# Fan-Luo/Legal-RAG

Hardware: AMD Instinct MI355X
Metric: queries/sec + Recall@10 (hybrid top-10) on UCC-en (higher is better)
Workload: dtype f32 dense (long batches: fp16 first pass, candidates re-scored in f32) / f64 bm25+fusion; 1 GPU; UCC-en 591 chunks, dense(768-d FlatIP)+BM25 hybrid fusion top-10 (BASELINE configs[1]); unique_queries=1168, top_k=10, fusion=rrf_norm_blend w=0.6/0.4 alpha=0.5 rrf_k=60 min_final=0.2

## Files before the change

legal-rag_amd/csrc/dense_tail.hip:

```cpp
#include "bm25_core.hpp"
#include "dense_dot.hpp"
#include "fuse_core.hpp"

#include <cfloat>
#include <cstdlib>

namespace amdr {

__global__ __launch_bounds__(64) void dense_select_fuse_kernel(amdr_fuse_params_t P, const float* __restrict__ S,
                                                               long ldS, long n, int nq, int kd, int cap,
                                                               float* __restrict__ fin_scores,
                                                               long long* __restrict__ fin_ids, ChanIn c0, ChanIn c1,
                                                               int max_out, long long* __restrict__ out_ids,
                                                               double* __restrict__ out_vals, int* __restrict__ out_mask,
                                                               int* __restrict__ out_count) {
  extern __shared__ __attribute__((aligned(16))) unsigned char smem[];
  C32* buf = reinterpret_cast<C32*>(smem);
  const int lane = threadIdx.x, sl = lane & 31;
  const int q = 2 * blockIdx.x + (lane >> 5);
  const bool has_q = q < nq;
  FusePre pre;
  pre.dense_bm25(c1, q, sl, has_q);
  C32 out = C32::pad();
  int got = select_row_pair_any(S, ldS, n, q, has_q, kd, lane, buf, out);
  if (got < 0) pair_rows_staged(S, ldS, n, 2 * blockIdx.x, nq, kd, cap, buf, lane, true, out, got);
  const bool v = sl < got;
  if (has_q && sl < kd) topk_store(out, v, sl, fin_scores + (size_t)q * kd, fin_ids + (size_t)q * kd);
  pre.dense(out, v);
  fuse_packed_body<32, true>(P, c0, c1, ChanIn::none(), nq, max_out, out_ids, out_vals, out_mask, out_count, pre, blockIdx.x * 2);
}

template <int V>
__device__ __forceinline__ int select_row_pair_margin(const float* __restrict__ S, long ldS, long n, int q, bool has_q, int k,
                                                      float margin, int lane, C32* scratch, C32& out, int& need) {
  const float* row = S + (size_t)q * ldS;
  const int j = lane & 31;
  f32x4 blk[V / 4];
#pragma unroll
  for (int u = 0; u < V / 4; ++u) {
    const long c0 = 128L * u + 4 * j;
    const f32x4 z = {0.f, 0.f, 0.f, 0.f};
    blk[u] = (has_q && c0 < ldS) ? __builtin_nontemporal_load(reinterpret_cast<const f32x4*>(row + c0)) : z;
  }
  u32 sk[V];
#pragma unroll
  for (int u = 0; u < V / 4; ++u)
#pragma unroll
    for (int e = 0; e < 4; ++e) {
      const long r = 128L * u + 4 * j + e;
      sk[4 * u + e] = (has_q && r < n) ? ord32(blk[u][e]) : 0u;
    }
  K32 lb;
  lb.c = 0u;
#pragma unroll
  for (int v = 0; v < V; ++v) lb.c = sk[v] > lb.c ? sk[v] : lb.c;
  const K32 sorted_best = wave_sortN_desc<K32, 32>(lb, lane);
  const int kk = (k - 1 < 31 ? k - 1 : 31);
  auto half_lane = [&](int x, int pos) -> int {
    const int a = __builtin_amdgcn_readlane(x, pos), b = __builtin_amdgcn_readlane(x, 32 + pos);
    return (lane & 32) ? b : a;
  };
  const u32 T = (u32)half_lane((int)sorted_best.c, kk);
  auto gather = [&](u32 Te, C32& c) -> int {
    int mine = 0;
#pragma unroll
    for (int v = 0; v < V; ++v) mine += (sk[v] >= Te) ? 1 : 0;
    int incl = mine;
    incl += __builtin_amdgcn_update_dpp(0, incl, 0x111, 0xf, 0xf, false);
    incl += __builtin_amdgcn_update_dpp(0, incl, 0x112, 0xf, 0xf, false);
    incl += __builtin_amdgcn_update_dpp(0, incl, 0x114, 0xf, 0xf, false);
    incl += __builtin_amdgcn_update_dpp(0, incl, 0x118, 0xf, 0xf, false);
    incl += __builtin_amdgcn_update_dpp(0, incl, 0x142, 0xa, 0xf, false);
    const int cnt = half_lane(incl, 31);
    if (cnt > 32) return -1;
    int at = (lane & 32) + incl - mine;
#pragma unroll
    for (int v = 0; v < V; ++v) {
      if (sk[v] >= Te) {
        C32 e;
        e.c = ((u64)sk[v] << 32) | (u64)(0xffffffffu - (u32)(128 * (v >> 2) + 4 * j + (v & 3)));
        scratch[at++] = e;
      }
    }
    wave_lds_fence();
    c = (j < cnt) ? scratch[lane] : C32::pad();
    c = wave_sortN_desc<C32, 32>(c, lane);
    wave_lds_fence();
    return cnt;
  };
  const u32 Te1 = T > 1u ? T : 1u;
  C32 c;
  int cnt = gather(Te1, c);
  if (cnt < 0) return -1;
  u32 cut = 1u;
  if (cnt > kk) {
    const float tk_f = __int_as_float(half_lane(__float_as_int(c.score()), kk));
    cut = ord32(tk_f - margin);
    cut = cut > 1u ? cut : 1u;
  }
  if (cut < Te1) {
    cnt = gather(cut, c);
    if (cnt < 0) return -1;
    need = cnt;
  } else {
    const unsigned long long m = __ballot(j < cnt && (u32)(c.c >> 32) >= cut);
    need = __popcll((lane & 32) ? (m >> 32) : (m & 0xffffffffull));
  }
  out = c;
  return cnt;
}

template <bool FUSE, int D128>
__global__ __launch_bounds__(64) void dense_hi_select_fuse_kernel(amdr_fuse_params_t P, const float* __restrict__ S, long ldS, long n,
                                                                  int nq, int kd, const float* __restrict__ X,
                                                                  const float* __restrict__ Q, int d,
                                                                  const float* __restrict__ eps, float margin_scale,
                                                                  float* __restrict__ fin_scores, long long* __restrict__ fin_ids,
                                                                  ChanIn c0, ChanIn c1, int max_out,
                                                                  long long* __restrict__ out_ids, double* __restrict__ out_vals,
                                                                  int* __restrict__ out_mask, int* __restrict__ out_count,
                                                                  unsigned int* __restrict__ fallbacks) {
  extern __shared__ __attribute__((aligned(16))) unsigned char smem[];
  C32* buf = reinterpret_cast<C32*>(smem);
  const int lane = threadIdx.x, sl = lane & 31, half = lane >> 5;
  const int q = 2 * blockIdx.x + half;
  const bool has_q = q < nq;
  FusePre pre;
  pre.have[0] = pre.have[1] = true;
  pre.have[2] = false;
  pre.id[1] = -1;
  pre.s[1] = 0.0;
  if (FUSE && has_q && sl < c1.k) {
    pre.id[1] = c1.ids[(size_t)q * c1.k + sl];
    pre.s[1] = chan_score(c1, q, sl);
  }
  const float e_q = has_q ? eps[q] : 0.f;
  const float margin = 2.f * e_q * margin_scale;
  bool exact_all = has_q && !(margin == margin && margin <= FLT_MAX);
  f32x4 qv[D128];
#pragma unroll
  for (int u = 0; u < D128; ++u) {
    const f32x4 z = {0.f, 0.f, 0.f, 0.f};
    qv[u] = has_q ? __builtin_nontemporal_load(reinterpret_cast<const f32x4*>(Q + (size_t)q * d + 128 * u + 4 * sl)) : z;
  }
  auto half_sum = [&](float v) -> float {
    v = dpp_add<0x111, 0xf>(v);
    v = dpp_add<0x112, 0xf>(v);
    v = dpp_add<0x114, 0xf>(v);
    v = dpp_add<0x118, 0xf>(v);
    v = dpp_add<0x142, 0xa>(v);
    const float s0 = __int_as_float(__builtin_amdgcn_readlane(__float_as_int(v), 31));
    const float s1 = __int_as_float(__builtin_amdgcn_readlane(__float_as_int(v), 63));
    return half ? s1 : s0;
  };
  auto row_load = [&](long r, f32x4 (&xv)[D128]) {
    const float* xr = X + (size_t)r * d + 4 * sl;
#pragma unroll
    for (int u = 0; u < D128; ++u) xv[u] = *reinterpret_cast<const f32x4*>(xr + 128 * u);
  };
  auto row_fma = [&](const f32x4 (&xv)[D128]) -> float {
    float acc = 0.f;
#pragma unroll
    for (int u = 0; u < D128; ++u)
#pragma unroll
      for (int e = 0; e < 4; ++e) acc = fmaf(xv[u][e], qv[u][e], acc);
    return half_sum(acc);
  };
  auto row_dot = [&](long r) -> float {
    f32x4 xv[D128];
    row_load(r, xv);
    return row_fma(xv);
  };
  C32 out = C32::pad();
  int need = 0, got = 0;
  {
    const float mg = (has_q && !exact_all) ? margin : 0.f;
    if (n <= 256)
      got = select_row_pair_margin<8>(S, ldS, n, q, has_q, kd, mg, lane, buf, out, need);
    else if (n <= 512)
      got = select_row_pair_margin<16>(S, ldS, n, q, has_q, kd, mg, lane, buf, out, need);
    else if (n <= 640)
      got = select_row_pair_margin<20>(S, ldS, n, q, has_q, kd, mg, lane, buf, out, need);
    else
      got = select_row_pair_margin<32>(S, ldS, n, q, has_q, kd, mg, lane, buf, out, need);
    exact_all = exact_all || (has_q && got < 0);
    if (exact_all) need = 0;
  }
  if (__any(exact_all)) {
    const unsigned long long fbm = __ballot(exact_all && sl == 0);
    if (lane == 0 && fallbacks) atomicAdd(fallbacks, (unsigned int)__popcll(fbm));
    const C32 keep = out;
    const int keep_need = need, keep_got = got;
    float* xs = const_cast<float*>(S);
    for (long r = 0; r < n; ++r) {
      const float v = row_dot(r);
      if (exact_all && sl == 0) xs[(size_t)q * ldS + r] = v;
    }
    __threadfence_block();
    C32 o2 = C32::pad();
    int g2 = select_row_pair_any(xs, ldS, n, q, has_q && exact_all, kd, lane, buf, o2);
    if (g2 < 0) pair_rows_staged(xs, ldS, n, 2 * blockIdx.x, nq, kd, 128, buf, lane, exact_all, o2, g2);
    if (exact_all) {
      out = o2;
      got = g2 < kd ? g2 : kd;
      need = 0;
    } else {
      out = keep;
      got = keep_got;
      need = keep_need;
    }
  }
  const int steps = __builtin_amdgcn_readfirstlane(max(__shfl(need, 0), __shfl(need, 32)));
  float mine_exact = 0.f;
  const int my_id = (int)out.id();
  for (int c = 0; c < steps; c += 2) {
    const int c1 = c + 1 < 32 ? c + 1 : 31;
    const int ra0 = __builtin_amdgcn_readlane(my_id, c), ra1 = __builtin_amdgcn_readlane(my_id, 32 + c);
    const int rb0 = __builtin_amdgcn_readlane(my_id, c1), rb1 = __builtin_amdgcn_readlane(my_id, 32 + c1);
    const bool la = c < need, lb = c + 1 < need;
    f32x4 xa[D128], xb[D128];
    row_load(la ? (long)(half ? ra1 : ra0) : 0, xa);
    row_load(lb ? (long)(half ? rb1 : rb0) : 0, xb);
    const float va = row_fma(xa), vb = row_fma(xb);
    if (la && sl == c) mine_exact = va;
    if (lb && sl == c + 1) mine_exact = vb;
  }
  if (need > 0) {
    C32 c = (sl < need) ? C32::make(mine_exact, (u32)out.id()) : C32::pad();
    c = wave_sortN_desc<C32, 32>(c, lane);
    out = c;
    got = need < kd ? need : kd;
  }
  const bool v = sl < got && sl < kd;
  if (has_q && sl < kd) topk_store(out, v, sl, fin_scores + (size_t)q * kd, fin_ids + (size_t)q * kd);
  if (FUSE) {
    pre.dense(out, v);
    fuse_packed_body<32, true>(P, c0, c1, ChanIn::none(), nq, max_out, out_ids, out_vals, out_mask, out_count, pre, blockIdx.x * 2);
  }
}

struct SmallArgs {
  const long long* term_ptr;
  const int* post_doc;
  const double* post_w;
  const double* idf;
  long n_terms, n_docs;
  const int* q_terms;
  const long long* q_ptr;
  int kb, cap, slab, use_select;
  double* bm_scores;
  long long* bm_ids;
  const float* X;
  const float* Q;
  long n_rows;
  int d, rows_per_block, blocks_per_query;
  float* S;
  long ldS;
  int kd, cap_sel;
  float* d_scores;
  long long* d_ids;
  int* ticket;
};

__device__ __forceinline__ int small_arrive(int* counter, int lane) {
  asm volatile("s_waitcnt vmcnt(0)" ::: "memory");
  int t = 0;
  if (lane == 0) {
    __builtin_amdgcn_fence(__ATOMIC_RELEASE, "agent");
    asm volatile("s_waitcnt vmcnt(0)" ::: "memory");
    t = __hip_atomic_fetch_add(counter, 1, __ATOMIC_RELAXED, __HIP_MEMORY_SCOPE_AGENT);
  }
  return __builtin_amdgcn_readfirstlane(t);
}
__device__ __forceinline__ void small_acquire(int* counter, int lane) {
  if (lane == 0) __hip_atomic_store(counter, 0, __ATOMIC_RELAXED, __HIP_MEMORY_SCOPE_AGENT);
  __builtin_amdgcn_fence(__ATOMIC_ACQUIRE, "agent");
  asm volatile("s_waitcnt vmcnt(0)" ::: "memory");
}

template <int NVT>
__global__ __launch_bounds__(256) void hybrid_small_kernel(SmallArgs A, amdr_fuse_params_t P, ChanIn c0, ChanIn c1, int nq,
                                                           int max_out, long long* __restrict__ out_ids,
                                                           double* __restrict__ out_vals, int* __restrict__ out_mask,
                                                           int* __restrict__ out_count) {
  extern __shared__ __attribute__((aligned(16))) unsigned char smem[];
  const int q = blockIdx.y, role = blockIdx.x;
  const int lane = threadIdx.x & 63, wave = threadIdx.x >> 6;
  int* rows_done = A.ticket + q;
  int* lists_done = A.ticket + 32 + q;
  const int sl = lane & 31;
  C32 dense_mine = C32::pad();
  bool have_dense = false, dense_valid = false;
  if (role == 0) {
    if (wave != 0) return;
    bm25_block_query<1, NVT>(A.term_ptr, A.post_doc, A.post_w, A.idf, A.n_terms, A.n_docs, A.q_terms, A.q_ptr, nq, A.kb,
                             A.cap, A.slab, A.use_select, nullptr, nullptr, A.bm_scores, A.bm_ids, q, 0, smem);
  } else {
    const long r0 = (long)(role - 1) * A.rows_per_block;
    long r1 = r0 + A.rows_per_block;
    if (r1 > A.n_rows) r1 = A.n_rows;
    for (long r = r0 + wave; r < r1; r += 4) {
      const float acc = dense_row_dot(A.X + (size_t)r * A.d, A.Q + (size_t)q * A.d, A.d, lane);
      if (lane == 63) A.S[(size_t)q * A.ldS + r] = acc;
    }
    asm volatile("s_waitcnt vmcnt(0)" ::: "memory");
    __syncthreads();
    if (wave != 0) return;
    if (small_arrive(rows_done, lane) != A.blocks_per_query - 2) return;
    small_acquire(rows_done, lane);
    C32* buf = reinterpret_cast<C32*>(smem);
    const float* row = A.S + (size_t)q * A.ldS;
    const long n = A.n_rows;
    WaveTopK<C32> tk;
    tk.init(buf, A.cap_sel, A.kd);
    const int got = select_row_any(row, 0, n, A.kd, lane, tk.buf);
    if (got >= 0)
      tk.cnt = got;
    else
      wave_topk_sweep(tk, row, 0, n, lane);
    wave_lds_fence();
    const bool v = lane < 32 && sl < tk.cnt;
    const C32 mine = v ? tk.buf[sl] : C32::pad();
    if (lane < A.kd) topk_store(mine, v, lane, A.d_scores + (size_t)q * A.kd, A.d_ids + (size_t)q * A.kd);
    dense_mine = mine;
    dense_valid = v;
    have_dense = true;
    wave_lds_fence();
  }
  if (small_arrive(lists_done, lane) != 1) return;
  small_acquire(lists_done, lane);
  long long dense_id = -1;
  double dense_s = 0.0;
  if (!have_dense && lane < 32 && sl < A.kd) {
    dense_id = A.d_ids[(size_t)q * A.kd + sl];
    dense_s = dense_id >= 0 ? (double)A.d_scores[(size_t)q * A.kd + sl] : 0.0;
  }
  FusePre pre;
  pre.dense_bm25(c1, q, sl, lane < 32);
  if (have_dense) {
    pre.dense(dense_mine, dense_valid);
  } else {
    pre.id[0] = dense_id;
    pre.s[0] = dense_s;
  }
  fuse_packed_body<32, true>(P, c0, c1, ChanIn::none(), q + 1, max_out, out_ids, out_vals, out_mask, out_count, pre, q);
}

bool dense_select_fuse_applies(long n, int slabs, int m, int kd, int kb) {
  const char* e = getenv("AMDR_DENSE_FUSE");
  if (e && e[0] == '0') return false;
  return slabs == 1 && n >= 1 && n <= 1024 && kd >= 1 && kd <= 32 && kb >= 0 && kd + kb <= 32 && m >= 1;
}

int dense_select_fuse_launch(const FuseTail& t, int q0, const float* S, long ldS, long n, int m, int kd, int cap,
                             float* fin_scores, int64_t* fin_ids, hipStream_t st) {
  const FuseTailArgs a = fuse_tail_args(t, q0, kd, nullptr, nullptr);
  hipLaunchKernelGGL(dense_select_fuse_kernel, dim3((m + 1) / 2), dim3(64), (size_t)cap * sizeof(C32), st, *t.p, S, ldS, n,
                     m, kd, cap, fin_scores, (long long*)fin_ids, a.c0, a.c1, a.mo, a.ids, a.vals, a.mask, a.count);
  AMDR_HIP(hipGetLastError());
  return AMDR_OK;
}

template <bool FUSE, class... Args>
static void hi_select_dispatch(int d, int m, size_t lds, hipStream_t st, Args... args) {
#define AMDR_HSF(D) \
  hipLaunchKernelGGL((dense_hi_select_fuse_kernel<FUSE, D>), dim3((m + 1) / 2), dim3(64), lds, st, args...)
  switch (d >> 7) {
    case 1: AMDR_HSF(1); break;
    case 2: AMDR_HSF(2); break;
    case 3: AMDR_HSF(3); break;
    case 4: AMDR_HSF(4); break;
    case 5: AMDR_HSF(5); break;
    case 6: AMDR_HSF(6); break;
    case 7: AMDR_HSF(7); break;
    default: AMDR_HSF(8); break;
  }
#undef AMDR_HSF
}

int dense_hi_select_launch(const FuseTail* t, int q0, const float* S, long ldS, long n, int m, int kd, const float* X,
                           const float* Q, int d, const float* eps, float* fin_scores, int64_t* fin_ids,
                           unsigned int* fallbacks, hipStream_t st) {
  const char* ms = getenv("AMDR_DENSE_SMALL_HI_MARGIN");
  const float margin_scale = ms ? (float)atof(ms) : 1.f;
  const size_t lds = 128 * sizeof(C32);
  const amdr_fuse_params_t P0{};
  const FuseTailArgs a = t ? fuse_tail_args(*t, q0, kd, nullptr, nullptr)
                           : FuseTailArgs{ChanIn::none(), ChanIn::none(), 0, nullptr, nullptr, nullptr, nullptr};
  if (t)
    hi_select_dispatch<true>(d, m, lds, st, *t->p, S, ldS, n, m, kd, X, Q, d, eps, margin_scale, fin_scores,
                             (long long*)fin_ids, a.c0, a.c1, a.mo, a.ids, a.vals, a.mask, a.count, fallbacks);
  else
    hi_select_dispatch<false>(d, m, lds, st, P0, S, ldS, n, m, kd, X, Q, d, eps, margin_scale, fin_scores,
                              (long long*)fin_ids, a.c0, a.c1, a.mo, a.ids, a.vals, a.mask, a.count, fallbacks);
  AMDR_HIP(hipGetLastError());
  return AMDR_OK;
}

bool hybrid_small_applies(long n_dense, long n_bm25, int nslabs, int nq, int kd, int kb) {
  const char* e = getenv("AMDR_HYBRID_SMALL");
  if (e && e[0] == '0') return false;
  return nq >= 1 && nq <= 4 && n_dense >= 1 && n_dense <= kSelectRowsMax && n_bm25 >= 1 && nslabs == 1 && kd >= 1 && kb >= 1 &&
         kd + kb <= 32;
}

static int hybrid_small_rows(long n, int nq) {
  static const int pinned = [] {
    const char* e = getenv("AMDR_HYBRID_SMALL_ROWS");
    int r = e ? atoi(e) : 0;
    if (r <= 0) return 0;
    if (r < 4) r = 4;
    if (r > 64) r = 64;
    return (r + 3) / 4 * 4;
  }();
  if (pinned) return pinned;
  return n * nq <= 2560 ? 16 : 32;
}

int hybrid_small_launch(const DenseRaw& dr, const Bm25Raw& br, const float* Q, const int* q_terms, const long long* q_ptr,
                        int nq, int kd, int kb, const amdr_fuse_params_t& P, const int64_t* dense_row2uid,
                        const int64_t* bm25_row2uid, float* dense_scores, int64_t* dense_ids, double* bm25_scores,
                        int64_t* bm25_ids, int64_t* out_ids, double* out_vals, int32_t* out_mask, int32_t* out_count,
                        hipStream_t st) {
  SmallArgs A;
  A.term_ptr = br.term_ptr;
  A.post_doc = br.post_doc;
  A.post_w = br.post_w;
  A.idf = br.idf;
  A.n_terms = br.n_terms;
  A.n_docs = br.n_docs;
  A.q_terms = q_terms;
  A.q_ptr = q_ptr;
  A.kb = kb;
  A.cap = br.cap;
  A.slab = br.slab;
  A.use_select = br.select_on ? 1 : 0;
  A.bm_scores = bm25_scores;
  A.bm_ids = (long long*)bm25_ids;
  A.X = dr.X;
  A.Q = Q;
  A.d = dr.d;
  A.n_rows = dr.n;
  A.rows_per_block = hybrid_small_rows(dr.n, nq);
  const int dense_blocks = (int)((dr.n + A.rows_per_block - 1) / A.rows_per_block);
  A.blocks_per_query = 1 + dense_blocks;
  A.S = dr.S;
  A.ldS = dr.ld;
  A.kd = kd;
  int cap_sel = topk_cap(kd);
  if (cap_sel < 128) cap_sel = 128;
  A.cap_sel = cap_sel;
  A.d_scores = dense_scores;
  A.d_ids = (long long*)dense_ids;
  A.ticket = br.ticket;
  size_t lds = br.lds;
  if (lds < (size_t)cap_sel * sizeof(C32)) lds = (size_t)cap_sel * sizeof(C32);
  const int mo = kd + kb;
  ChanIn c0{nullptr, nullptr, (const long long*)dense_row2uid, kd, 0};
  ChanIn c1{(const long long*)bm25_ids, (const void*)bm25_scores, (const long long*)bm25_row2uid, kb, 1};
#define AMDR_HS_LAUNCH(NVT)                                                                                        \
  hipLaunchKernelGGL((hybrid_small_kernel<NVT>), dim3(A.blocks_per_query, nq), dim3(256), lds, st, A, P, c0, c1, nq, mo, \
                     (long long*)out_ids, out_vals, out_mask, out_count)
  const int nv = br.nvt;
  if (nv <= 4) AMDR_HS_LAUNCH(4);
  else if (nv <= 8) AMDR_HS_LAUNCH(8);
  else if (nv <= 10) AMDR_HS_LAUNCH(10);
  else if (nv <= 16) AMDR_HS_LAUNCH(16);
  else if (nv <= 20) AMDR_HS_LAUNCH(20);
  else AMDR_HS_LAUNCH(32);
#undef AMDR_HS_LAUNCH
  AMDR_HIP(hipGetLastError());
  return AMDR_OK;
}

}

using namespace amdr;

extern "C" {

int amdr_hybrid_small_device(amdr_dense_t* dense, amdr_bm25_t* bm25, const float* Q_dev, const int32_t* q_terms_dev,
                             const int64_t* q_ptr_dev, int32_t nq, int32_t kd, int32_t kb, const amdr_fuse_params_t* p,
                             const int64_t* dense_row2uid, const int64_t* bm25_row2uid, float* dense_scores_dev,
                             int64_t* dense_ids_dev, double* bm25_scores_dev, int64_t* bm25_ids_dev, int64_t* out_ids,
                             double* out_vals, int32_t* out_mask, int32_t* out_count, void* stream) {
  AMDR_REQUIRE(dense && bm25, "hybrid_small: null index handle");
  AMDR_REQUIRE(p != nullptr, "hybrid_small: null params");
  AMDR_REQUIRE(p->method >= 0 && p->method <= AMDR_FUSE_WEIGHTED_SUM, "hybrid_small: method=%d", p->method);
  AMDR_REQUIRE(nq >= 0 && kd >= 1 && kd <= AMDR_MAX_K && kb >= 1 && kb <= AMDR_MAX_K, "hybrid_small: bad sizes");
  if (nq == 0) return AMDR_OK;
  AMDR_REQUIRE(Q_dev && q_terms_dev && q_ptr_dev, "hybrid_small: null query buffers");
  AMDR_REQUIRE(dense_scores_dev && dense_ids_dev && bm25_scores_dev && bm25_ids_dev, "hybrid_small: null channel lists");
  AMDR_REQUIRE(out_ids && out_vals && out_mask && out_count, "hybrid_small: null output");
  int64_t nd = 0, nb = 0;
  int rc;
  if ((rc = amdr_dense_ntotal(dense, &nd))) return rc;
  if ((rc = amdr_bm25_ndocs(bm25, &nb))) return rc;
  AMDR_REQUIRE(kd <= nd || nd == 0, "hybrid_small: kd=%d > %lld rows", kd, (long long)nd);
  bool one = false;
  if (nd >= 1 && nb >= 1 && nq <= 4 && dense_device_of(dense) >= 0) {
    std::lock_guard<std::mutex> gd(dense_mutex(dense));
    std::lock_guard<std::mutex> gb(bm25_mutex(bm25));
    AMDR_HIP(hipSetDevice(dense_device_of(dense)));
    Bm25Raw br;
    if ((rc = bm25_small_raw(bm25, nq, kb, &br))) return rc;
    if (hybrid_small_applies((long)nd, (long)nb, br.nslabs, nq, kd, kb)) {
      DenseRaw dr;
      if ((rc = dense_small_raw(dense, nq, &dr))) return rc;
      one = true;
      rc = hybrid_small_launch(dr, br, Q_dev, q_terms_dev, (const long long*)q_ptr_dev, nq, kd, kb, *p, dense_row2uid,
                               bm25_row2uid, dense_scores_dev, dense_ids_dev, bm25_scores_dev, bm25_ids_dev, out_ids,
                               out_vals, out_mask, out_count, (hipStream_t)stream);
    }
  }
  if (one) return rc;
  if ((rc = amdr_bm25_search_device(bm25, q_terms_dev, q_ptr_dev, nq, kb, bm25_scores_dev, bm25_ids_dev, stream))) return rc;
  return amdr_dense_search_fuse_device(dense, Q_dev, nq, kd, p, dense_row2uid, bm25_ids_dev, bm25_scores_dev, kb,
                                       bm25_row2uid, dense_scores_dev, dense_ids_dev, out_ids, out_vals, out_mask,
                                       out_count, stream);
}

}
```

legal-rag_amd/csrc/fuse_core.hpp:

```cpp
#pragma once
#include "common.hpp"
#include "topk.hpp"

#include <cmath>

namespace amdr {

__device__ __forceinline__ double wave_min(double v) { return wave_allmin_f64(v); }
__device__ __forceinline__ double wave_max(double v) { return wave_allmax_f64(v); }
__device__ __forceinline__ void lds_sync() {
  __builtin_amdgcn_fence(__ATOMIC_ACQ_REL, "wavefront");
  __builtin_amdgcn_wave_barrier();
}

struct ChanIn {
  const long long* ids;
  const void* scores;
  const long long* row2uid;
  int k;
  int is_f64;
  __host__ __device__ static ChanIn none() { return ChanIn{nullptr, nullptr, nullptr, 0, 0}; }
};

__device__ __forceinline__ double chan_score(const ChanIn& c, int qi, int j) {
  size_t off = (size_t)qi * c.k + j;
  return c.is_f64 ? ((const double*)c.scores)[off] : (double)((const float*)c.scores)[off];
}
__device__ __forceinline__ long long chan_uid(const ChanIn& c, int qi, int j) {
  long long id = c.ids[(size_t)qi * c.k + j];
  if (id >= 0 && c.row2uid) id = c.row2uid[id];
  return id;
}

struct FuseCtx {
  double rmn, rmx;
  bool rdeg, wrrf;
  double w[3], lo[3], hi[3];
};
template <class ScoreAt>
__device__ __forceinline__ void fuse_eval(const amdr_fuse_params_t& P, const FuseCtx& X, double t, const int (&pos)[3],
                                          ScoreAt&& score_at, double (&val)[AMDR_FUSE_NVALS], int& mk) {
  const double rrf_norm = X.rdeg ? 0.0 : (t - X.rmn) / (X.rmx - X.rmn);
  double nrm[3], raw[3], wt[3];
  mk = 0;
#pragma unroll
  for (int c = 0; c < 3; ++c) {
    const int p = pos[c];
    nrm[c] = 0.0;
    raw[c] = 0.0;
    if (p >= 0) {
      mk |= (1 << c);
      const double s = score_at(c, p);
      nrm[c] = (X.hi[c] - X.lo[c] < 1e-12) ? 0.0 : (s - X.lo[c]) / (X.hi[c] - X.lo[c]);
      const double wc = X.wrrf ? X.w[c] : 1.0;
      raw[c] = wc * (1.0 / (double)(P.rrf_k + p + 1));
    }
    wt[c] = X.w[c] * nrm[c];
  }
  const double wsum = (wt[0] + wt[1]) + wt[2];
  double score, con[3] = {0.0, 0.0, 0.0};
  if (P.method == AMDR_FUSE_WEIGHTED_SUM) {
    score = wsum;
#pragma unroll
    for (int c = 0; c < 3; ++c) con[c] = wt[c];
  } else if (P.method == AMDR_FUSE_RRF || P.method == AMDR_FUSE_WRRF) {
    score = rrf_norm;
    const double mass = score;
    if (!(mass <= 0.0 || t <= 1e-18)) {
#pragma unroll
      for (int c = 0; c < 3; ++c)
        if (pos[c] >= 0) con[c] = mass * raw[c] / t;
    }
  } else {
    score = P.alpha * rrf_norm + (1.0 - P.alpha) * wsum;
#pragma unroll
    for (int c = 0; c < 3; ++c) con[c] = 0.0 + (1.0 - P.alpha) * wt[c];
    const double mass = P.alpha * rrf_norm;
    if (!(mass <= 0.0 || t <= 1e-18)) {
#pragma unroll
      for (int c = 0; c < 3; ++c)
        if (pos[c] >= 0) con[c] = con[c] + mass * raw[c] / t;
    }
  }
  val[AMDR_FV_SCORE] = score;
  val[AMDR_FV_RRF_NORM] = rrf_norm;
  val[AMDR_FV_WSUM] = wsum;
  val[AMDR_FV_NORM_DENSE] = nrm[0];
  val[AMDR_FV_NORM_BM25] = nrm[1];
  val[AMDR_FV_NORM_COLBERT] = nrm[2];
  val[AMDR_FV_CONTRIB_DENSE] = con[0];
  val[AMDR_FV_CONTRIB_BM25] = con[1];
  val[AMDR_FV_CONTRIB_COLBERT] = con[2];
}

struct FusePre {
  bool have[3];
  long long id[3];
  double s[3];
  __device__ __forceinline__ void dense_bm25(const ChanIn& c1, int q, int sl, bool live) {
    have[0] = have[1] = true;
    have[2] = false;
    id[1] = -1;
    s[1] = 0.0;
    if (live && sl < c1.k) {
      id[1] = c1.ids[(size_t)q * c1.k + sl];
      s[1] = chan_score(c1, q, sl);
    }
  }
  __device__ __forceinline__ void dense(const C32& c, bool valid) {
    id[0] = valid ? c.id() : -1ll;
    s[0] = valid ? (double)c.score() : 0.0;
  }
  __device__ __forceinline__ void bm25(const C64& c, bool valid) {
    id[1] = valid ? c.idv : -1ll;
    s[1] = valid ? unord64(c.key) : 0.0;
  }
};
template <int W, bool PRE>
__device__ __forceinline__ void fuse_packed_body(const amdr_fuse_params_t& P, const ChanIn& c0, const ChanIn& c1,
                                                 const ChanIn& c2, int nq, int max_out, long long* __restrict__ out_ids,
                                                 double* __restrict__ out_vals, int* __restrict__ out_mask,
                                                 int* __restrict__ out_count, const FusePre& pre, int qbase) {
  constexpr int G = 64 / W;
  __shared__ long long s_uid[G][W];
  __shared__ double s_sc[G][W];
  __shared__ double s_chs[G][3][W];
  __shared__ int s_pos[G][3][W];
  const int lane = threadIdx.x, seg = lane / W, sl = lane % W;
  const int qi = qbase + seg;
  const bool live = qi < nq;
  const ChanIn ch[3] = {c0, c1, c2};
  const double w[3] = {P.w_dense, P.w_bm25, P.w_colbert};
  const unsigned long long seg_bits = (W == 64) ? ~0ull : (((1ull << (W & 63)) - 1ull) << (seg * W));
  long long* uid = s_uid[seg];
  double* sc = s_sc[seg];

  int n[3] = {0, 0, 0};
  double lo[3] = {INFINITY, INFINITY, INFINITY}, hi[3] = {-INFINITY, -INFINITY, -INFINITY};
  long long my_uid[3] = {-1, -1, -1};
#pragma unroll
  for (int c = 0; c < 3; ++c) {
    if (ch[c].k == 0) continue;
    const int j = sl;
    const bool inr = live && j < ch[c].k;
    long long id = -1;
    double s = 0.0;
    if (PRE && pre.have[c]) {
      if (inr) {
        id = pre.id[c];
        s = pre.s[c];
      }
    } else if (inr) {
      id = ch[c].ids[(size_t)qi * ch[c].k + j];
      s = chan_score(ch[c], qi, j);
    }
    const bool has = inr && id >= 0;
    if (!has) s = 0.0;
    if (has && ch[c].row2uid) id = ch[c].row2uid[id];
    my_uid[c] = has ? id : -1;
    s_chs[seg][c][sl] = s;
    const unsigned long long hm = __ballot(has) & seg_bits;
    n[c] = __popcll(hm);
    const double nxt = __shfl_down(s, 1);
    const bool in_order = !(has && sl + 1 < n[c]) || s >= nxt;
    const bool prefix = hm == (seg_bits & ((n[c] >= 64 ? ~0ull : ((1ull << n[c]) - 1ull)) << (seg * W)));
    if (__ballot(!in_order || !prefix) == 0ull) {
      const int first = seg * W, last = seg * W + (n[c] > 0 ? n[c] - 1 : 0);
      const double top = __shfl(s, first), bot = __shfl(s, last);
      hi[c] = n[c] > 0 ? top : -(double)INFINITY;
      lo[c] = n[c] > 0 ? bot : (double)INFINITY;
    } else {
      lo[c] = seg_allmin_f64<W>(has ? s : (double)INFINITY);
      hi[c] = seg_allmax_f64<W>(has ? s : -(double)INFINITY);
    }
  }

  int U = 0;
#pragma unroll
  for (int c = 0; c < 3; ++c) {
    if (ch[c].k == 0) continue;
    const int U0 = U;
    const bool v = sl < n[c];
    const long long my = my_uid[c];
    int f = -1;
    int u_end = 0;
#pragma unroll
    for (int g = 0; g < G; ++g) {
      const int ug = __builtin_amdgcn_readlane(U0, g * W);
      u_end = ug > u_end ? ug : u_end;
    }
    for (int u0 = 0; u0 < u_end; u0 += 4) {
      long long e[4];
#pragma unroll
      for (int i = 0; i < 4; ++i) e[i] = uid[(u0 + i) & (W - 1)];
#pragma unroll
      for (int i = 0; i < 4; ++i) f = (u0 + i < U0 && e[i] == my) ? u0 + i : f;
    }
    f = v ? f : -1;
    const bool isnew = v && f < 0;
    const unsigned long long m = __ballot(isnew) & seg_bits;
    const unsigned long long lt = m & ((1ull << lane) - 1ull);
    const int idx = isnew ? U + __popcll(lt) : f;
    if (isnew) {
      uid[idx] = my;
      s_pos[seg][0][idx] = -1;
      s_pos[seg][1][idx] = -1;
      s_pos[seg][2][idx] = -1;
    }
    lds_sync();
    if (v) s_pos[seg][c][idx] = sl;
    U += __popcll(m);
    lds_sync();
  }

  const bool wrrf = (P.method == AMDR_FUSE_WRRF);
  const int u = sl;
  const bool act = u < U;
  int pp[3] = {-1, -1, -1};
  double t = 0.0;
  if (act) {
#pragma unroll
    for (int c = 0; c < 3; ++c) {
      pp[c] = s_pos[seg][c][u];
      if (pp[c] >= 0) {
        const double wc = wrrf ? w[c] : 1.0;
        const double v = wc * (1.0 / (double)(P.rrf_k + pp[c] + 1));
        t = t + v;
      }
    }
  }
  FuseCtx X;
  X.rmn = seg_allmin_f64<W>(act ? t : (double)INFINITY);
  X.rmx = seg_allmax_f64<W>(act ? t : -(double)INFINITY);
  X.rdeg = (X.rmx - X.rmn < 1e-12);
  X.wrrf = wrrf;
#pragma unroll
  for (int c = 0; c < 3; ++c) {
    X.w[c] = w[c];
    X.lo[c] = lo[c];
    X.hi[c] = hi[c];
  }

  double val[AMDR_FUSE_NVALS];
  int mk = 0;
  if (act) {
    fuse_eval(P, X, t, pp, [&](int c, int p) { return s_chs[seg][c][p]; }, val, mk);
    sc[u] = val[AMDR_FV_SCORE];
  }
  lds_sync();
  int kept = 0;
  const size_t obase = (size_t)qi * max_out;
  if (act) {
    const double s = val[AMDR_FV_SCORE];
    int r = 0;
    for (int v2 = 0; v2 < U; ++v2) {
      const double o = sc[v2];
      r += (o > s) || (o == s && v2 < u);
    }
    if (s >= P.min_final_score) kept = 1;
    out_ids[obase + r] = uid[u];
    out_mask[obase + r] = mk;
#pragma unroll
    for (int x = 0; x < AMDR_FUSE_NVALS; ++x) out_vals[(obase + r) * AMDR_FUSE_NVALS + x] = val[x];
  } else if (live && u < max_out) {
    out_ids[obase + u] = -1;
    out_mask[obase + u] = 0;
#pragma unroll
    for (int x = 0; x < AMDR_FUSE_NVALS; ++x) out_vals[(obase + u) * AMDR_FUSE_NVALS + x] = 0.0;
  }
  kept = __popcll(__ballot(kept != 0) & seg_bits);
  if (live && sl == 0) out_count[qi] = kept;
}

struct FuseTailArgs {
  ChanIn c0, c1;
  int mo;
  long long* ids;
  double* vals;
  int* mask;
  int* count;
};
inline FuseTailArgs fuse_tail_args(const FuseTail& t, int q0, int kd, const float* dense_scores, const int64_t* dense_ids) {
  const int mo = kd + t.kb;
  return FuseTailArgs{ChanIn{(const long long*)dense_ids, dense_scores, (const long long*)t.dense_row2uid, kd, 0},
                      ChanIn{(const long long*)(t.kb ? t.bm25_ids + (size_t)q0 * t.kb : nullptr),
                             t.kb ? (const void*)(t.bm25_scores + (size_t)q0 * t.kb) : nullptr,
                             (const long long*)t.bm25_row2uid, t.kb, 1},
                      mo, (long long*)(t.out_ids + (size_t)q0 * mo), t.out_vals + (size_t)q0 * mo * AMDR_FUSE_NVALS,
                      t.out_mask + (size_t)q0 * mo, t.out_count + q0};
}

}
```

Before: 155.8 million queries/s.

## Use DPP half-wave bitonic sorts with adaptive width and cheaper exact rescoring

```diff
diff --git a/legal-rag_amd/csrc/check_pair_sort_width.cpp b/legal-rag_amd/csrc/check_pair_sort_width.cpp
--- /dev/null
+++ b/legal-rag_amd/csrc/check_pair_sort_width.cpp
@@ -0,0 +1,81 @@
+#include "pair_sort_width.hpp"
+
+#include <algorithm>
+#include <cstdint>
+#include <cstdio>
+#include <functional>
+#include <vector>
+
+using namespace amdr;
+
+typedef uint64_t u64;
+
+static void network(std::vector<u64>& v, int N) {
+  for (int size = 2; size <= N; size <<= 1)
+    for (int stride = size >> 1; stride > 0; stride >>= 1) {
+      std::vector<u64> o(64);
+      for (int lane = 0; lane < 64; ++lane) o[lane] = v[lane ^ stride];
+      for (int lane = 0; lane < 64; ++lane) {
+        const bool keep_better = bitonic_keeps_better(lane, size, stride, N);
+        const bool mine_better = v[lane] > o[lane];
+        v[lane] = (keep_better == mine_better) ? v[lane] : o[lane];
+      }
+    }
+}
+
+static u64 rng_state = 0x9e3779b97f4a7c15ull;
+static u64 rnd() {
+  rng_state ^= rng_state << 13;
+  rng_state ^= rng_state >> 7;
+  rng_state ^= rng_state << 17;
+  return rng_state;
+}
+
+int main() {
+  long cases = 0, narrow = 0;
+  for (int rep = 0; rep < 8; ++rep)
+    for (int c0 = 0; c0 <= 32; ++c0)
+      for (int c1 = 0; c1 <= 32; ++c1) {
+        const int cnt[2] = {c0, c1};
+        std::vector<u64> v(64, 0ull);
+        std::vector<u64> want[2];
+        for (int h = 0; h < 2; ++h) {
+          std::vector<uint32_t> ids(32);
+          for (int i = 0; i < 32; ++i) ids[i] = (uint32_t)i * 37u + (uint32_t)h;
+          for (int i = 31; i > 0; --i) std::swap(ids[i], ids[rnd() % (u64)(i + 1)]);
+          for (int i = 0; i < cnt[h]; ++i) {
+            const u64 score = 1ull + rnd() % (rep < 4 ? 4ull : 1000ull);
+            const u64 key = (score << 32) | (u64)(0xffffffffu - ids[i]);
+            v[32 * h + i] = key;
+            want[h].push_back(key);
+          }
+          std::sort(want[h].begin(), want[h].end(), std::greater<u64>());
+        }
+        bool wide = false;
+        for (int lane = 0; lane < 64; ++lane) wide = wide || pair_sort_lane_wide(lane & 31, cnt[lane >> 5]);
+        if (wide != (c0 > 16 || c1 > 16)) {
+          printf("FAIL vote: counts %d %d -> %s\n", c0, c1, wide ? "wide" : "narrow");
+          return 1;
+        }
+        std::vector<u64> got = v, got32 = v;
+        network(got, wide ? 32 : 16);
+        network(got32, 32);
+        if (got != got32) {
+          printf("FAIL counts %d %d: the voted width and the 32-lane network differ\n", c0, c1);
+          return 1;
+        }
+        for (int h = 0; h < 2; ++h)
+          for (int i = 0; i < 32; ++i) {
+            const u64 w = i < cnt[h] ? want[h][(size_t)i] : 0ull;
+            if (got[32 * h + i] != w) {
+              printf("FAIL counts %d %d: half %d lane %d holds %llx, std::sort says %llx\n", c0, c1, h, i,
+                     (unsigned long long)got[32 * h + i], (unsigned long long)w);
+              return 1;
+            }
+          }
+        ++cases;
+        narrow += wide ? 0 : 1;
+      }
+  printf("pair sort width ok: %ld cases, %ld on the 16-lane network\n", cases, narrow);
+  return 0;
+}
diff --git a/legal-rag_amd/csrc/dense_tail.hip b/legal-rag_amd/csrc/dense_tail.hip
--- a/legal-rag_amd/csrc/dense_tail.hip
+++ b/legal-rag_amd/csrc/dense_tail.hip
@@ -1,6 +1,7 @@
 #include "bm25_core.hpp"
 #include "dense_dot.hpp"
 #include "fuse_core.hpp"
+#include "pair_sort_width.hpp"
 
 #include <cfloat>
 #include <cstdlib>
@@ -30,6 +31,57 @@
   fuse_packed_body<32, true>(P, c0, c1, ChanIn::none(), nq, max_out, out_ids, out_vals, out_mask, out_count, pre, blockIdx.x * 2);
 }
 
+template <int S>
+__device__ __forceinline__ u32 row_xor(u32 x) {
+  static_assert(S == 1 || S == 2 || S == 4 || S == 8, "stride inside a row of 16");
+  if constexpr (S == 1) {
+    return (u32)__builtin_amdgcn_mov_dpp((int)x, 0xB1, 0xf, 0xf, true);
+  } else if constexpr (S == 2) {
+    return (u32)__builtin_amdgcn_mov_dpp((int)x, 0x4E, 0xf, 0xf, true);
+  } else if constexpr (S == 4) {
+    const int t = __builtin_amdgcn_mov_dpp((int)x, 0x104, 0xf, 0x5, false);
+    return (u32)__builtin_amdgcn_update_dpp(t, (int)x, 0x114, 0xf, 0xa, false);
+  } else {
+    return (u32)__builtin_amdgcn_mov_dpp((int)x, 0x128, 0xf, 0xf, true);
+  }
+}
+template <int S>
+__device__ __forceinline__ K32 pair_xchg(const K32& v) {
+  K32 o;
+  if constexpr (S == 16)
+    o.c = lane_xor_sw(v.c, 16);
+  else
+    o.c = row_xor<S>(v.c);
+  return o;
+}
+template <int S>
+__device__ __forceinline__ C32 pair_xchg(const C32& v) {
+  C32 o;
+  if constexpr (S == 16)
+    o.c = lane_xor_sw(v.c, 16);
+  else
+    o.c = ((u64)row_xor<S>((u32)(v.c >> 32)) << 32) | row_xor<S>((u32)v.c);
+  return o;
+}
+template <int N, int SIZE, int STRIDE, class C>
+__device__ __forceinline__ C pair_sort_steps(C v, int lane) {
+  if constexpr (SIZE > N) {
+    return v;
+  } else {
+    const C o = pair_xchg<STRIDE>(v);
+    v = (bitonic_keeps_better(lane, SIZE, STRIDE, N) == better(v, o)) ? v : o;
+    if constexpr (STRIDE > 1)
+      return pair_sort_steps<N, SIZE, STRIDE / 2>(v, lane);
+    else
+      return pair_sort_steps<N, SIZE * 2, SIZE>(v, lane);
+  }
+}
+template <int N, class C>
+__device__ __forceinline__ C pair_sort_desc(C v, int lane) {
+  static_assert(N == 16 || N == 32, "half-wave lists");
+  return pair_sort_steps<N, 2, 1>(v, lane);
+}
+
 template <int V>
 __device__ __forceinline__ int select_row_pair_margin(const float* __restrict__ S, long ldS, long n, int q, bool has_q, int k,
                                                       float margin, int lane, C32* scratch, C32& out, int& need) {
@@ -54,14 +106,14 @@
   lb.c = 0u;
 #pragma unroll
   for (int v = 0; v < V; ++v) lb.c = sk[v] > lb.c ? sk[v] : lb.c;
-  const K32 sorted_best = wave_sortN_desc<K32, 32>(lb, lane);
+  const K32 sorted_best = pair_sort_desc<32>(lb, lane);
   const int kk = (k - 1 < 31 ? k - 1 : 31);
   auto half_lane = [&](int x, int pos) -> int {
     const int a = __builtin_amdgcn_readlane(x, pos), b = __builtin_amdgcn_readlane(x, 32 + pos);
     return (lane & 32) ? b : a;
   };
   const u32 T = (u32)half_lane((int)sorted_best.c, kk);
-  auto gather = [&](u32 Te, C32& c) -> int {
+  auto gather = [&](u32 Te, bool sorted, C32& c) -> int {
     int mine = 0;
 #pragma unroll
     for (int v = 0; v < V; ++v) mine += (sk[v] >= Te) ? 1 : 0;
@@ -73,24 +125,30 @@
     incl += __builtin_amdgcn_update_dpp(0, incl, 0x142, 0xa, 0xf, false);
     const int cnt = half_lane(incl, 31);
     if (cnt > 32) return -1;
-    int at = (lane & 32) + incl - mine;
+    C32* slot = scratch + ((lane & 32) + incl - mine);
+    const u32 nid0 = 0xffffffffu - 4u * (u32)j;
 #pragma unroll
     for (int v = 0; v < V; ++v) {
       if (sk[v] >= Te) {
         C32 e;
-        e.c = ((u64)sk[v] << 32) | (u64)(0xffffffffu - (u32)(128 * (v >> 2) + 4 * j + (v & 3)));
-        scratch[at++] = e;
+        e.c = ((u64)sk[v] << 32) | (u64)(nid0 - (u32)(128 * (v >> 2) + (v & 3)));
+        *slot++ = e;
       }
     }
     wave_lds_fence();
     c = (j < cnt) ? scratch[lane] : C32::pad();
-    c = wave_sortN_desc<C32, 32>(c, lane);
+    if (sorted) {
+      if (__ballot(pair_sort_lane_wide(j, cnt)) == 0ull)
+        c = pair_sort_desc<16>(c, lane);
+      else
+        c = pair_sort_desc<32>(c, lane);
+    }
     wave_lds_fence();
     return cnt;
   };
   const u32 Te1 = T > 1u ? T : 1u;
   C32 c;
-  int cnt = gather(Te1, c);
+  int cnt = gather(Te1, true, c);
   if (cnt < 0) return -1;
   u32 cut = 1u;
   if (cnt > kk) {
@@ -99,7 +157,7 @@
     cut = cut > 1u ? cut : 1u;
   }
   if (cut < Te1) {
-    cnt = gather(cut, c);
+    cnt = gather(cut, false, c);
     if (cnt < 0) return -1;
     need = cnt;
   } else {
@@ -109,6 +167,8 @@
   out = c;
   return cnt;
 }
+
+extern "C" __device__ int amdr_writelane_i32(int val, int lane, int old) __asm("llvm.amdgcn.writelane.i32");
 
 template <bool FUSE, int D128>
 __global__ __launch_bounds__(64) void dense_hi_select_fuse_kernel(amdr_fuse_params_t P, const float* __restrict__ S, long ldS, long n,
@@ -143,12 +203,15 @@
     const f32x4 z = {0.f, 0.f, 0.f, 0.f};
     qv[u] = has_q ? __builtin_nontemporal_load(reinterpret_cast<const f32x4*>(Q + (size_t)q * d + 128 * u + 4 * sl)) : z;
   }
-  auto half_sum = [&](float v) -> float {
+  auto half_sum_ends = [&](float v) -> float {
     v = dpp_add<0x111, 0xf>(v);
     v = dpp_add<0x112, 0xf>(v);
     v = dpp_add<0x114, 0xf>(v);
     v = dpp_add<0x118, 0xf>(v);
-    v = dpp_add<0x142, 0xa>(v);
+    asm("s_nop 1\n\tv_add_f32_dpp %0, %0, %0 row_bcast:15 row_mask:0xa bank_mask:0xf" : "+v"(v));
+    return v;
+  };
+  auto half_ends_to_all = [&](float v) -> float {
     const float s0 = __int_as_float(__builtin_amdgcn_readlane(__float_as_int(v), 31));
     const float s1 = __int_as_float(__builtin_amdgcn_readlane(__float_as_int(v), 63));
     return half ? s1 : s0;
@@ -158,18 +221,18 @@
 #pragma unroll
     for (int u = 0; u < D128; ++u) xv[u] = *reinterpret_cast<const f32x4*>(xr + 128 * u);
   };
-  auto row_fma = [&](const f32x4 (&xv)[D128]) -> float {
+  auto row_fma_ends = [&](const f32x4 (&xv)[D128]) -> float {
     float acc = 0.f;
 #pragma unroll
     for (int u = 0; u < D128; ++u)
 #pragma unroll
       for (int e = 0; e < 4; ++e) acc = fmaf(xv[u][e], qv[u][e], acc);
-    return half_sum(acc);
+    return half_sum_ends(acc);
   };
   auto row_dot = [&](long r) -> float {
     f32x4 xv[D128];
     row_load(r, xv);
-    return row_fma(xv);
+    return half_ends_to_all(row_fma_ends(xv));
   };
   C32 out = C32::pad();
   int need = 0, got = 0;
@@ -211,23 +274,39 @@
     }
   }
   const int steps = __builtin_amdgcn_readfirstlane(max(__shfl(need, 0), __shfl(need, 32)));
-  float mine_exact = 0.f;
+  const bool wide_final = __ballot(pair_sort_lane_wide(sl, need)) != 0ull;
   const int my_id = (int)out.id();
+  const int need0 = __builtin_amdgcn_readlane(need, 0), need1 = __builtin_amdgcn_readlane(need, 32);
+  int lane_late = lane;
+  asm volatile("" : "+v"(lane_late));
+  const u32 lane_bytes = 16u * (u32)(lane_late & 31), half_shift = (u32)(lane_late & 32) >> 1;
+  const u32 pitch = 4u * (u32)d;
+  const char* Xb = reinterpret_cast<const char*>(X);
+  auto row_load_pair = [&](u32 r0, u32 r1, f32x4 (&xv)[D128]) {
+    const u32 r = ((r0 | (r1 << 16)) >> half_shift) & 0xffffu;
+    const u32 off = __umul24(r, pitch) + lane_bytes;
+    const char* xr = Xb + (size_t)off;
+#pragma unroll
+    for (int u = 0; u < D128; ++u) xv[u] = *reinterpret_cast<const f32x4*>(xr + 512 * u);
+  };
+  int mine_bits = 0;
   for (int c = 0; c < steps; c += 2) {
     const int c1 = c + 1 < 32 ? c + 1 : 31;
-    const int ra0 = __builtin_amdgcn_readlane(my_id, c), ra1 = __builtin_amdgcn_readlane(my_id, 32 + c);
-    const int rb0 = __builtin_amdgcn_readlane(my_id, c1), rb1 = __builtin_amdgcn_readlane(my_id, 32 + c1);
-    const bool la = c < need, lb = c + 1 < need;
+    const u32 ra0 = (u32)__builtin_amdgcn_readlane(my_id, c), ra1 = (u32)__builtin_amdgcn_readlane(my_id, 32 + c);
+    const u32 rb0 = (u32)__builtin_amdgcn_readlane(my_id, c1), rb1 = (u32)__builtin_amdgcn_readlane(my_id, 32 + c1);
     f32x4 xa[D128], xb[D128];
-    row_load(la ? (long)(half ? ra1 : ra0) : 0, xa);
-    row_load(lb ? (long)(half ? rb1 : rb0) : 0, xb);
-    const float va = row_fma(xa), vb = row_fma(xb);
-    if (la && sl == c) mine_exact = va;
-    if (lb && sl == c + 1) mine_exact = vb;
-  }
+    row_load_pair(c < need0 ? ra0 : 0u, c < need1 ? ra1 : 0u, xa);
+    row_load_pair(c + 1 < need0 ? rb0 : 0u, c + 1 < need1 ? rb1 : 0u, xb);
+    const int va = __float_as_int(row_fma_ends(xa)), vb = __float_as_int(row_fma_ends(xb));
+    mine_bits = amdr_writelane_i32(__builtin_amdgcn_readlane(va, 31), c, mine_bits);
+    mine_bits = amdr_writelane_i32(__builtin_amdgcn_readlane(va, 63), 32 + c, mine_bits);
+    mine_bits = amdr_writelane_i32(__builtin_amdgcn_readlane(vb, 31), c1, mine_bits);
+    mine_bits = amdr_writelane_i32(__builtin_amdgcn_readlane(vb, 63), 32 + c1, mine_bits);
+  }
+  const float mine_exact = __int_as_float(mine_bits);
   if (need > 0) {
     C32 c = (sl < need) ? C32::make(mine_exact, (u32)out.id()) : C32::pad();
-    c = wave_sortN_desc<C32, 32>(c, lane);
+    c = wide_final ? pair_sort_desc<32>(c, lane) : pair_sort_desc<16>(c, lane);
     out = c;
     got = need < kd ? need : kd;
   }
diff --git a/legal-rag_amd/csrc/fuse_core.hpp b/legal-rag_amd/csrc/fuse_core.hpp
--- a/legal-rag_amd/csrc/fuse_core.hpp
+++ b/legal-rag_amd/csrc/fuse_core.hpp
@@ -37,9 +37,9 @@
   bool rdeg, wrrf;
   double w[3], lo[3], hi[3];
 };
-template <class ScoreAt>
+template <class ScoreAt, class RecipAt>
 __device__ __forceinline__ void fuse_eval(const amdr_fuse_params_t& P, const FuseCtx& X, double t, const int (&pos)[3],
-                                          ScoreAt&& score_at, double (&val)[AMDR_FUSE_NVALS], int& mk) {
+                                          ScoreAt&& score_at, RecipAt&& recip_at, double (&val)[AMDR_FUSE_NVALS], int& mk) {
   const double rrf_norm = X.rdeg ? 0.0 : (t - X.rmn) / (X.rmx - X.rmn);
   double nrm[3], raw[3], wt[3];
   mk = 0;
@@ -53,7 +53,7 @@
       const double s = score_at(c, p);
       nrm[c] = (X.hi[c] - X.lo[c] < 1e-12) ? 0.0 : (s - X.lo[c]) / (X.hi[c] - X.lo[c]);
       const double wc = X.wrrf ? X.w[c] : 1.0;
-      raw[c] = wc * (1.0 / (double)(P.rrf_k + p + 1));
+      raw[c] = wc * recip_at(c, p);
     }
     wt[c] = X.w[c] * nrm[c];
   }
@@ -91,6 +91,12 @@
   val[AMDR_FV_CONTRIB_DENSE] = con[0];
   val[AMDR_FV_CONTRIB_BM25] = con[1];
   val[AMDR_FV_CONTRIB_COLBERT] = con[2];
+}
+
+template <class ScoreAt>
+__device__ __forceinline__ void fuse_eval(const amdr_fuse_params_t& P, const FuseCtx& X, double t, const int (&pos)[3],
+                                          ScoreAt&& score_at, double (&val)[AMDR_FUSE_NVALS], int& mk) {
+  fuse_eval(P, X, t, pos, score_at, [&](int, int p) { return 1.0 / (double)(P.rrf_k + p + 1); }, val, mk);
 }
 
 struct FusePre {
@@ -213,10 +219,13 @@
     lds_sync();
   }
 
+  sc[sl] = 1.0 / (double)(P.rrf_k + sl + 1);
+  lds_sync();
   const bool wrrf = (P.method == AMDR_FUSE_WRRF);
   const int u = sl;
   const bool act = u < U;
   int pp[3] = {-1, -1, -1};
+  double rr[3] = {0.0, 0.0, 0.0};
   double t = 0.0;
   if (act) {
 #pragma unroll
@@ -224,11 +233,13 @@
       pp[c] = s_pos[seg][c][u];
       if (pp[c] >= 0) {
         const double wc = wrrf ? w[c] : 1.0;
-        const double v = wc * (1.0 / (double)(P.rrf_k + pp[c] + 1));
+        rr[c] = sc[pp[c]];
+        const double v = wc * rr[c];
         t = t + v;
       }
     }
   }
+  lds_sync();
   FuseCtx X;
   X.rmn = seg_allmin_f64<W>(act ? t : (double)INFINITY);
   X.rmx = seg_allmax_f64<W>(act ? t : -(double)INFINITY);
@@ -244,7 +255,7 @@
   double val[AMDR_FUSE_NVALS];
   int mk = 0;
   if (act) {
-    fuse_eval(P, X, t, pp, [&](int c, int p) { return s_chs[seg][c][p]; }, val, mk);
+    fuse_eval(P, X, t, pp, [&](int c, int p) { return s_chs[seg][c][p]; }, [&](int c, int) { return rr[c]; }, val, mk);
     sc[u] = val[AMDR_FV_SCORE];
   }
   lds_sync();
diff --git a/legal-rag_amd/csrc/pair_sort_width.hpp b/legal-rag_amd/csrc/pair_sort_width.hpp
--- /dev/null
+++ b/legal-rag_amd/csrc/pair_sort_width.hpp
@@ -0,0 +1,17 @@
+#pragma once
+
+#if defined(__HIPCC__) || defined(__CUDACC__)
+#define AMDR_HD __host__ __device__
+#else
+#define AMDR_HD
+#endif
+
+namespace amdr {
+
+AMDR_HD constexpr bool pair_sort_lane_wide(int sl, int cnt) { return sl >= 16 && sl < cnt; }
+
+AMDR_HD constexpr bool bitonic_keeps_better(int lane, int size, int stride, int N) {
+  return ((size == N) || (lane & size) == 0) == ((lane & stride) == 0);
+}
+
+}
```

After: 156.8 million queries/s (median of 6 runs). Within noise of the previous version (+0.7%).
